# bennevans/mjrl

Measured on AMD Instinct MI355X. Metric: NPG train_step timesteps/sec, Humanoid 1M-step batch @ 1/2/4/8 MI355X, higher is better.
Workload: dtype f32 (split-f16 MFMA, f32 accumulate); 1 GPU; humanoid_npg_1M; obs_dim=376, act_dim=17, algo=npg, horizon=1000, cg_iters=10, parallelism=dp1, comm=LocalComm

## Files before the change

### include/mjrl_amd.h

```cpp
#ifndef MJRL_AMD_H
#define MJRL_AMD_H

#include <stdint.h>

#ifdef __cplusplus
extern "C" {
#endif

#define MJRL_OK 0
#define MJRL_EINVAL (-1)
#define MJRL_ESHAPE (-2)

typedef struct mjrl_shape {
    int32_t n, m;
    int32_t h0, h1;
    int32_t np, mp;
    int32_t d;
    int32_t packed;
} mjrl_shape;

typedef struct mjrl_rows {
    int64_t T;
    const float* xhat;
    const float* act;
// ... 88 lines not shown
int mjrl_quadratic_baseline_gram_scratch(int32_t n, int64_t T, int64_t* doubles);
int mjrl_quadratic_baseline_gram(const double* obs, const double* returns, int64_t T, int32_t n,
                                 const int64_t* path_off, int64_t P, double* scratch, double* out, void* stream);
int mjrl_quadratic_baseline_gram_f32(const float* obs, const float* obs_lo, const double* returns, int64_t T,
                                     int32_t n, const int64_t* path_off, int64_t P, double* scratch, double* out,
                                     void* stream);
int mjrl_quadratic_baseline_residual(const double* obs, const double* returns, int64_t T, int32_t n,
                                     const int64_t* path_off, int64_t P, const double* coeffs, double* scratch,
                                     double* out, void* stream);
int mjrl_quadratic_baseline_residual_f32(const float* obs, const float* obs_lo, const double* returns, int64_t T,
                                         int32_t n, const int64_t* path_off, int64_t P, const double* coeffs,
                                         double* scratch, double* out, void* stream);

int mjrl_gather_rows(const void* src, int64_t row_bytes, const int64_t* idx, int64_t n, void* dst,
                     void* stream);

int mjrl_moments(const double* x, int64_t N, const double* center, double* rpart,
                 double* out, void* stream);
int mjrl_moments_f32(const float* x, int64_t N, const double* center, double* rpart,
                     double* out, void* stream);

#define MJRL_MOM_SCRATCH 2056
int mjrl_moments2(const double* x1, int64_t N1, const double* c1, const double* x2, int64_t N2,
                  const double* c2, double* rpart, double* out1, double* out2, void* stream);
int mjrl_whiten_moments(const double* adv, int64_t T, const double* m1, const double* m2, double eps,
                        float* adv32, double* w64, double* rpart, double* out, void* stream);

int mjrl_moments_combine(const double* gathered, int32_t world, int32_t rec, int32_t ngroups, double* out,
                         void* stream);

int mjrl_whiten(const double* adv, int64_t T, const double* m1, const double* m2,
                double eps, float* adv32, double* w64, void* stream);

int mjrl_dapg_adv(const double* w64, int64_t T, const double* mw1, const double* mw2,
                  int64_t T_demo, double demo_coef, float* adv_vpg, void* stream);

int mjrl_pack_params(const mjrl_shape* s, const float* theta, float* packed,
                     int32_t clamp_log_std, float min_log_std, void* stream);

int mjrl_policy_vpg(const mjrl_shape* s, const mjrl_rows* rows, const float* packed_theta,
                    const float* out_shift, const float* out_scale,
                    const mjrl_scratch* sc, float* gsum, void* stream);
int mjrl_policy_fvp(const mjrl_shape* s, const mjrl_rows* rows, int64_t T_fvp,
                    const float* packed_theta, const float* packed_v,
                    const float* out_scale, const mjrl_scratch* sc, const int32_t* done,
                    float* gsum, void* stream);
int mjrl_policy_eval(const mjrl_shape* s, const mjrl_rows* rows, int64_t T_eval,
                     const float* packed_theta_new, const float* packed_theta_old,
                     const float* out_shift, const float* out_scale,
                     const mjrl_scratch* sc, double* sums, void* stream);
int mjrl_policy_eval_if(const mjrl_shape* s, const mjrl_rows* rows, int64_t T_eval, const float* packed_theta_new,
                        const float* packed_theta_old, const float* out_shift, const float* out_scale,
                        const mjrl_scratch* sc, double* sums, const int32_t* skip, void* stream);

int mjrl_vpg_accumulate(const mjrl_shape* s, const mjrl_rows* rows, const float* packed_theta,
                        const float* out_shift, const float* out_scale, const mjrl_scratch* sc,
                        void* stream);
int mjrl_vpg_accumulate_pack(const mjrl_shape* s, const mjrl_rows* rows, const float* obs,
                             const float* packed_theta, const float* out_shift, const float* out_scale,
                             const mjrl_scratch* sc, void* stream);
int mjrl_policy_vpg_pack(const mjrl_shape* s, const mjrl_rows* rows, const float* obs,
                         const float* packed_theta, const float* out_shift, const float* out_scale,
                         const mjrl_scratch* sc, float* gsum, void* stream);
int mjrl_fvp_accumulate(const mjrl_shape* s, const mjrl_rows* rows, int64_t T_fvp,
                        const float* packed_theta, const float* packed_v, const float* out_scale,
                        const int32_t* done, const mjrl_scratch* sc, void* stream);
int mjrl_gather_grads(const mjrl_shape* s, const mjrl_rows* rows, int64_t T,
                      const mjrl_scratch* sc, int32_t with_log_std, const int32_t* done,
                      float* gsum, void* stream);
int mjrl_fused_path(const mjrl_shape* s);

#define MJRL_CG_STATE 4096
int mjrl_cg_init(const mjrl_shape* s, const float* b, float* x, float* r, float* p,
                 float* packed_p, float* cg, int32_t* done, void* stream);
int mjrl_cg_init_scaled(const mjrl_shape* s, const float* gsum, double scale, float* g, float* x, float* r, float* p,
                        float* packed_p, float* cg, int32_t* done, void* stream);
int mjrl_cg_step(const mjrl_shape* s, const float* gsum, double inv_T, float damping,
                 const float* packed_theta, float* x, float* r, float* p, float* z,
                 float* packed_p, float* cg, int32_t* done, float residual_tol,
                 void* stream);

int mjrl_gather_cg_z(const mjrl_shape* s, const mjrl_rows* rows, int64_t T, const mjrl_scratch* sc,
                     const int32_t* done, float* gsum, double inv_T, float damping,
                     const float* packed_theta, const float* p, float* z, float* cg, void* stream);
int mjrl_cg_step_xr_p(const mjrl_shape* s, float* x, const float* r, float* r_out, float* p,
                      const float* z, float* packed_p, float* cg, int32_t* done, float residual_tol,
                      void* stream);

int mjrl_cg_z(const mjrl_shape* s, const float* gsum, double inv_T, float damping, const float* packed_theta,
              const float* p, float* z, float* cg, const int32_t* done, void* stream);

int mjrl_cg_step1(const mjrl_shape* s, const float* gsum, double inv_T, float damping,
                  const float* packed_theta, float* x, const float* r, float* r_out, const float* p,
                  float* p_out, float* packed_p, float* cg, int32_t* done, float residual_tol,
                  void* stream);

int mjrl_cg_init_vec(int32_t d, const float* b, float* x, float* r, float* p, float* cg,
                     int32_t* done, void* stream);
int mjrl_cg_update(int32_t d, const float* z, float* x, float* r, float* p, float* cg,
                   int32_t* done, float residual_tol, void* stream);

int mjrl_scale_vec(const float* gsum, int32_t d, double scale, float* g, void* stream);

#define MJRL_STEP_OUT 1024
int mjrl_npg_step(const mjrl_shape* s, const float* g, const float* x, const float* theta,
                  int32_t mode, float delta, float alpha_in, int32_t const_lr,
// ... 78 lines not shown
```

### mjrl_amd/_lib.py

```python
import ctypes as C
import os

import torch

HERE = os.path.dirname(os.path.abspath(__file__))
LIB_PATH = os.path.join(HERE, "lib", "libmjrl_amd.so")

MJRL_OK = 0
MJRL_EINVAL = -1
MJRL_ESHAPE = -2
CG_STATE = 4096
CG_PZ_PARTS = 1024
STEP_OUT = 1024
LS_LOG, LS_STATE = 32, 128
MOM_SCRATCH = 2056


class Shape(C.Structure):
    _fields_ = [("n", C.c_int32), ("m", C.c_int32), ("h0", C.c_int32), ("h1", C.c_int32),
                ("np", C.c_int32), ("mp", C.c_int32), ("d", C.c_int32), ("packed", C.c_int32)]


class Rows(C.Structure):
    _fields_ = [("T", C.c_int64)] + [(k, C.c_void_p) for k in (
# ... 12 lines not shown
    _fields_ = [("p", C.c_void_p * 7), ("exp_avg", C.c_void_p * 7), ("exp_avg_sq", C.c_void_p * 7)]


class PolicyFitData(C.Structure):
    _fields_ = [(k, C.c_void_p) for k in ("obs", "act", "adv", "ll_old", "old_log_std", "in_shift", "in_scale",
                                          "out_shift", "out_scale")] + \
               [("T", C.c_int64), ("n", C.c_int32), ("m", C.c_int32), ("h0", C.c_int32), ("h1", C.c_int32),
                ("kind", C.c_int32), ("clip", C.c_double)]


POLICY_FIT_BC, POLICY_FIT_PPO = 0, 1


class Adam(C.Structure):
    _fields_ = [("lr", C.c_double), ("beta1", C.c_double), ("beta2", C.c_double), ("eps", C.c_double),
                ("weight_decay", C.c_double), ("step0", C.c_int64)]


P = C.c_void_p
I32 = C.c_int32
I64 = C.c_int64
F32 = C.c_float
F64 = C.c_double
SP = C.POINTER(Shape)

SIGNATURES = {
    "mjrl_shape_init": [SP, I32, I32, I32, I32],
    "mjrl_scratch_size": [SP, I64, C.POINTER(I64), C.POINTER(I64), C.POINTER(I32)],
    "mjrl_pack_batch": [P, P, I64, SP, P, P, P, P, P],
    "mjrl_obs_colscale": [P, I64, SP, P, P, P, P],
    "mjrl_obs_colscale_f32": [P, I64, SP, P, P, P, P],
    "mjrl_obs_colscale_range": [P, P, SP, P, P, P, P],
    "mjrl_pack_batch_split": [P, P, I64, SP, P, P, P, P, P, P, P],
    "mjrl_pack_batch_f32": [P, P, I64, SP, P, P, P, P, P],
    "mjrl_pack_batch_split_f32": [P, P, I64, SP, P, P, P, P, P, P, P],
    "mjrl_split_supported": [SP],
    "mjrl_gae": [P, P, P, P, I64, F64, F64, I32, P, P, P, P],
    "mjrl_gae_wave": [P, P, P, P, I64, F64, F64, I32, P, P, P, P],
    "mjrl_gae_scan": [P, P, P, P, I64, F64, F64, I32, P, P, P, P],
    "mjrl_linear_baseline": [P, I64, I32, P, I64, P, P, P],
    "mjrl_linear_baseline_f32": [P, I64, I32, P, I64, P, P, P],
    "mjrl_moments": [P, I64, P, P, P, P],
    "mjrl_moments_f32": [P, I64, P, P, P, P],
    "mjrl_moments2": [P, I64, P, P, I64, P, P, P, P, P],
    "mjrl_whiten_moments": [P, I64, P, P, F64, P, P, P, P, P],
    "mjrl_moments_combine": [P, I32, I32, I32, P, P],
    "mjrl_whiten": [P, I64, P, P, F64, P, P, P],
    "mjrl_dapg_adv": [P, I64, P, P, I64, F64, P, P],
    "mjrl_pack_params": [SP, P, P, I32, F32, P],
    "mjrl_policy_vpg": [SP, C.POINTER(Rows), P, P, P, C.POINTER(Scratch), P, P],
    "mjrl_policy_fvp": [SP, C.POINTER(Rows), I64, P, P, P, C.POINTER(Scratch), P, P, P],
    "mjrl_policy_eval": [SP, C.POINTER(Rows), I64, P, P, P, P, C.POINTER(Scratch), P, P],
    "mjrl_policy_eval_if": [SP, C.POINTER(Rows), I64, P, P, P, P, C.POINTER(Scratch), P, P, P],
    "mjrl_vpg_accumulate": [SP, C.POINTER(Rows), P, P, P, C.POINTER(Scratch), P],
    "mjrl_vpg_accumulate_pack": [SP, C.POINTER(Rows), P, P, P, P, C.POINTER(Scratch), P],
    "mjrl_policy_vpg_pack": [SP, C.POINTER(Rows), P, P, P, P, C.POINTER(Scratch), P, P],
    "mjrl_fvp_accumulate": [SP, C.POINTER(Rows), I64, P, P, P, P, C.POINTER(Scratch), P],
    "mjrl_gather_grads": [SP, C.POINTER(Rows), I64, C.POINTER(Scratch), I32, P, P, P],
    "mjrl_fused_path": [SP],
    "mjrl_cg_init": [SP, P, P, P, P, P, P, P, P],
    "mjrl_cg_init_scaled": [SP, P, F64, P, P, P, P, P, P, P, P],
    "mjrl_cg_step": [SP, P, F64, F32, P, P, P, P, P, P, P, P, F32, P],
    "mjrl_gather_cg_z": [SP, C.POINTER(Rows), I64, C.POINTER(Scratch), P, P, F64, F32, P, P, P, P, P],
    "mjrl_cg_step_xr_p": [SP, P, P, P, P, P, P, P, P, F32, P],
    "mjrl_cg_z": [SP, P, F64, F32, P, P, P, P, P, P],
    "mjrl_cg_step1": [SP, P, F64, F32, P, P, P, P, P, P, P, P, P, F32, P],
    "mjrl_cg_init_vec": [I32, P, P, P, P, P, P, P],
    "mjrl_cg_update": [I32, P, P, P, P, P, P, F32, P],
    "mjrl_scale_vec": [P, I32, F64, P, P],
    "mjrl_gather_rows": [P, I64, P, I64, P, P],
    "mjrl_linear_baseline_gram_scratch": [I32, I64, C.POINTER(I64)],
    "mjrl_linear_baseline_gram": [P, P, I64, I32, P, I64, P, P, P],
    "mjrl_linear_baseline_residual": [P, P, I64, I32, P, I64, P, P, P, P],
    "mjrl_linear_baseline_gram_f32": [P, P, I64, I32, P, I64, P, P, P],
    "mjrl_linear_baseline_residual_f32": [P, P, I64, I32, P, I64, P, P, P, P],
    "mjrl_linear_baseline_gram_f32x2": [P, P, P, I64, I32, P, I64, P, P, P],
    "mjrl_linear_baseline_residual_f32x2": [P, P, P, I64, I32, P, I64, P, P, P, P],
    "mjrl_quadratic_baseline_gram_scratch": [I32, I64, C.POINTER(I64)],
    "mjrl_quadratic_baseline_gram": [P, P, I64, I32, P, I64, P, P, P],
    "mjrl_quadratic_baseline_gram_f32": [P, P, P, I64, I32, P, I64, P, P, P],
    "mjrl_quadratic_baseline_residual": [P, P, I64, I32, P, I64, P, P, P, P],
    "mjrl_quadratic_baseline_residual_f32": [P, P, P, I64, I32, P, I64, P, P, P, P],
    "mjrl_npg_step": [SP, P, P, P, I32, F32, F32, I32, F32, P, P, P, P],
    "mjrl_trpo_trial": [SP, P, P, F32, P, P, P, P, F64, F64, I32, I32, P, P, P],
    "mjrl_policy_mean": [SP, P, I64, P, P, P, P, P, P, P],
    "mjrl_policy_mean_slots": [SP, P, P, I64, I64, P, P, P, P, P, P, P],
    "mjrl_value_features_slots": [P, P, P, I64, I64, I32, I64, P, P],
    "mjrl_value_features_finish": [P, P, I64, I32, I64, I64, P, P, P],
    "mjrl_value_mlp_scratch": [I32, I32, C.POINTER(I64)],
    "mjrl_value_mlp_epoch": [P, P, I64, I32, P, I64, I32, C.POINTER(ValueNet), C.POINTER(Adam), P, P, P, P],
    "mjrl_policy_fit_scratch": [I32, I32, I32, I32, I32, C.POINTER(I64)],
    "mjrl_policy_fit_epoch": [C.POINTER(PolicyFitData), P, I64, I32, C.POINTER(PolicyNet), C.POINTER(Adam), P, I32,
                              P, P, P],
    "mjrl_build_flags": [],
    "mjrl_host_stage_f64": [P, I64, I32, P, P, P],
    "mjrl_host_stage_f32": [P, I64, I32, P, P, P],
    "mjrl_host_stage_paths_f64": [P, P, I32, I32, P, P, P],
    "mjrl_host_stage_paths_f64x": [P, P, I32, I32, P, P, P, P, P, I32, P],
    "mjrl_host_stage_lo_paths_f64": [P, P, I32, I32, P],
    "mjrl_host_extras_portable": [P, I64, I32, P, P, P],
    "mjrl_host_stage_rows_f64x": [P, I64, I32, P, P, P, P, P, P, P],
    "mjrl_host_stage_f64_portable": [P, I64, I32, P, P, P],
    "mjrl_host_stage_avx512": [],
    "mjrl_host_gather": [P, P, I32, P],
}

# ... 13 lines not shown
    if not os.path.isabs(path) and not os.path.exists(path):
        path = os.path.join(os.path.dirname(HERE), path)
    if not os.path.exists(path):
        raise MjrlError("mjrl_amd HIP library not built: %s (run `python -m mjrl_amd.build`)" % path)
    lib = C.CDLL(path)
    for name, args in SIGNATURES.items():
        fn = getattr(lib, name)
        fn.argtypes = args
        fn.restype = C.c_int
    if lib.mjrl_build_flags() & BUILD_ABLATION and os.environ.get("MJRL_AMD_ALLOW_ABLATION") != "1":
        raise MjrlError("%s is a timing-ablation build (MJRL_KX_ABL_*: its results are wrong by construction); "
                        "set MJRL_AMD_ALLOW_ABLATION=1 to load it for timing" % path)
    _LIB = lib
    return lib


STAGE_LIB_PATH = os.path.join(HERE, "lib", "libmjrl_stage.so")
STAGE_FUNCS = ("mjrl_host_stage_f64", "mjrl_host_stage_f32", "mjrl_host_stage_paths_f64",
               "mjrl_host_stage_paths_f64x", "mjrl_host_stage_lo_paths_f64", "mjrl_host_extras_portable",
               "mjrl_host_stage_rows_f64x",
               "mjrl_host_stage_f64_portable", "mjrl_host_stage_avx512", "mjrl_host_gather")
_STAGE = None


def stage_lib():
    global _STAGE
    if _STAGE is None:
        if not os.path.exists(STAGE_LIB_PATH):
            raise MjrlError("mjrl_amd staging library not built: %s (run `python -m mjrl_amd.build`)"
                            % STAGE_LIB_PATH)
        lib = C.CDLL(STAGE_LIB_PATH)
        for name in STAGE_FUNCS:
            fn = getattr(lib, name)
            fn.argtypes = SIGNATURES[name]
            fn.restype = C.c_int
        _STAGE = lib
    return _STAGE


def lib():
    if not torch.cuda.is_available():
        raise MjrlError("mjrl_amd needs an AMD GPU (torch.cuda.is_available() is False); "
                        "there is no CPU fallback")
    return load()


def check(rc, what):
    if rc != MJRL_OK:
        msg = {MJRL_EINVAL: "invalid argument", MJRL_ESHAPE: "unsupported policy shape"}.get(
            rc, "HIP error %d" % rc)
        raise MjrlError("%s failed: %s" % (what, msg))


QUERIES = ("mjrl_fused_path", "mjrl_split_supported", "mjrl_build_flags", "mjrl_host_stage_avx512")
_CALLS = {}


class _DevPtr:

    @staticmethod
    def from_param(v, _T=torch.Tensor, _vp=C.c_void_p):
        if type(v) is _T:
            return _vp(v.data_ptr())
        if v is None or type(v) is _vp:
            return v
        if isinstance(v, _T):
            return _vp(v.data_ptr())
        return _vp.from_param(v)


class _HostPtr:

    @staticmethod
    def from_param(v, _vp=C.c_void_p):
        c = getattr(v, "ctypes", None)
        return _vp(c.data) if c is not None else _DevPtr.from_param(v)


def _errcheck(rc, fn, args):
    if rc:
        check(rc, fn.__name__)
    return rc


def _checked(path, names, ptr):
    h = _CALLS.get(path)
    if h is None:
        h = _CALLS[path] = C.CDLL(path)
        for name in names:
            fn = getattr(h, name)
            fn.argtypes = [ptr if a is P else a for a in SIGNATURES[name]]
            fn.restype = C.c_int
            if name not in QUERIES:
                fn.errcheck = _errcheck
    return h


def calls(loader=lib):
    return _checked(loader()._name, SIGNATURES, _DevPtr)


def stage_calls():
    return _checked(stage_lib()._name, STAGE_FUNCS, _HostPtr)


def make_shape(n, m, h0, h1, loader=load):
    s = Shape()
# ... 13 lines not shown
```

### mjrl_amd/csrc/policy.hip

```cpp
#include <math.h>
#include <stdlib.h>

#include "common.h"

using namespace mjrl;

namespace {

enum { FWD = 0, FVP = 1, EVAL = 2 };

struct RowArgs {
    int64_t T;
    int np, m;
    const float* xhat;
    const float* act;
    const float* adv;
    const float* adv_vpg;
    float* a0;
    float* a1;
    float* mu0;
    float* ll0;
    float* gu0;
    float* gu1;
    float* gp;
// ... 961 lines not shown
        const int s0 = w * per, s1 = min(S, s0 + per);
        const float* p = wpart + (int64_t)blockIdx.x * S * 64 + lane;
        if (s1 > s0) MJRL_SLAB_CHECK((int64_t)blockIdx.x * S * 64 + lane + (int64_t)(s1 - 1) * 64, wcap);
        for (int sb = s0; sb < s1; sb += GATHER_PER) {
            float v[GATHER_PER];
#pragma unroll
            for (int j = 0; j < GATHER_PER; ++j) v[j] = sb + j < s1 ? p[(int64_t)(sb + j) * 64] : 0.f;
#pragma unroll
            for (int j = 0; j < GATHER_PER; ++j) acc += (double)v[j];
        }
    } else if (f < d && lspart) {
        const int lsj = f - d_mu;
        const int per = (G + GATHER_WAVES - 1) / GATHER_WAVES;
        const int b0 = w * per, b1 = min(G, b0 + per);
        for (int b = b0; b < b1; ++b) acc += lspart[(int64_t)b * mp + lsj];
    }
    part[w][lane] = acc;
    if (done && *done) return;
    __syncthreads();
    if (w == 0) {
        float gs = 0.f;
        if (f < d) {
            double t = part[0][lane];
#pragma unroll
            for (int j = 1; j < GATHER_WAVES; ++j) t += part[j][lane];
            gs = (float)t;
            gsum[f] = gs;
        }
        if (cz.p) cgz_epilogue(cz, f, d, gs, pf, lsv);
    }
}

__global__ void __launch_bounds__(64) k_eval_final(const double* __restrict__ rpart, int G, double* __restrict__ sums,
                                                   const int32_t* __restrict__ skip) {
    if (skip && *skip) return;
    double s = 0.0, k = 0.0;
    for (int b = threadIdx.x; b < G; b += 64) {
        s += rpart[2 * b];
        k += rpart[2 * b + 1];
    }
    s = wave_sum(s);
    k = wave_sum(k);
    if (threadIdx.x == 0) {
        sums[0] = s;
        sums[1] = k;
    }
}

}

#include "fused.h"
#include "ks.h"
#include "kx.h"

namespace {

constexpr int ROW_GRID_CAP = 512;
constexpr int WGRAD_SLICES_CAP = 128;

inline int bt_for(int h0, int h1) { return rows_bt(h0 > h1 ? h0 : h1); }

inline int row_grid(const mjrl_shape* s, int64_t T) {
    const int bt = bt_for(s->h0, s->h1);
    int64_t nt = (T + bt - 1) / bt;
    if (nt < 1) nt = 1;
    return (int)(nt < ROW_GRID_CAP ? nt : ROW_GRID_CAP);
}

inline int wgrad_slices(int64_t T) {
    int64_t nt = (T + WT - 1) / WT;
    if (nt < 1) nt = 1;
    return (int)(nt < WGRAD_SLICES_CAP ? nt : WGRAD_SLICES_CAP);
}

struct JobSet {
    int njobs;
    WJob job[3];
    int64_t floats;
};

int64_t slab_floats(const mjrl_shape* s, int S);

JobSet make_jobs(const mjrl_shape* s, const mjrl_rows* r, int S) {
    JobSet js{};
    auto add = [&](const float* G, int ldg, const float* A, int lda, int N, int K, int bias) {
        WJob& j = js.job[js.njobs++];
        j.G = G; j.ldg = ldg; j.A = A; j.lda = lda; j.N = N; j.K = K;
        j.nbN = (N + WB - 1) / WB; j.nbK = (K + WB - 1) / WB; j.bias = bias;
        j.off = js.floats;
        js.floats += (int64_t)S * N * K;
        j.boff = js.floats;
        if (bias) js.floats += (int64_t)S * N;
    };
    if (s->h0 == 0) {
        add(r ? r->gp : nullptr, s->mp, r ? r->xhat : nullptr, s->np, s->mp, s->np, 0);
    } else {
        add(r ? r->gu0 : nullptr, s->h0, r ? r->xhat : nullptr, s->np, s->h0, s->np, 0);
        add(r ? r->gu1 : nullptr, s->h1, r ? r->a0 : nullptr, s->h0, s->h1, s->h0, 1);
        add(r ? r->gp : nullptr, s->mp, r ? r->a1 : nullptr, s->h1, s->mp, s->h1, 1);
    }
    return js;
}

template <int H0, int H1, int MP, int MODE>
int launch_rows_t(const RowArgs& ra, int grid, hipStream_t st) {
    using L = Layout<H0, H1, MP>;
// ... 83 lines not shown
    static const bool v = getenv("MJRL_AMD_WGRAD_OLD") && getenv("MJRL_AMD_WGRAD_OLD")[0] == '1';
    return v;
}
bool wall_supported(const mjrl_shape* s) {
    if (wall_off() || s->h0 == 0 || s->h0 != s->h1 || s->np % 16 || !wall_npbm(s)) return false;
    if (s->mp != 16 && s->mp != 32 && s->mp != 64) return false;
    if (s->h0 == 128 && s->mp == 64 && wall_npbm(s) == 8) return false;
    return s->h0 == 128 || ((s->h0 == 32 || s->h0 == 64) && s->mp == 64);
}
inline int wall_cap(const mjrl_shape*) { return 256; }
inline int wall_slices(const mjrl_shape* s, int64_t T) {
    const int bt = 32;
    int64_t tiles = (T + bt - 1) / bt;
    if (tiles < 1) tiles = 1;
    const int cap = wall_cap(s);
    const int64_t tps = (tiles + cap - 1) / cap;
    return (int)((tiles + tps - 1) / tps);
}
inline int rows_slices(const mjrl_shape* s, int64_t T) { return wall_supported(s) ? wall_slices(s, T) : wgrad_slices(T); }

inline int grad_slices(const mjrl_shape* s, int64_t T) {
    const int p = acc_path(s, T);
    return p == 2 ? ks_grid(T) : (p == 1 ? fused_grid(T) : rows_slices(s, T));
}

bool ksx_supported(const mjrl_shape* s) { return ks_supported(s) && s->np % 128 == 0; }

template <int MP, int KG, int MODE>
int launch_ks_t(const RowArgs& ra, const FOut& fo, int grid, hipStream_t st) {
    using L = KLayout<MP, KG>;
    auto fn = k_ks<MP, KG, MODE>;
    static bool attr = false;
    if (!attr) {
        hipError_t e = hipFuncSetAttribute((const void*)fn, hipFuncAttributeMaxDynamicSharedMemorySize, L::bytes);
        if (e != hipSuccess) return (int)e;
        attr = true;
    }
    hipLaunchKernelGGL(fn, dim3(grid), dim3(KT), L::bytes, st, ra, fo);
    return (int)hipGetLastError();
}

template <int MP, int KG, int MODE, bool PACK = false>
int launch_kx_t(const RowArgs& ra, const FOut& fo, int grid, hipStream_t st) {
    using L = XLayout<MP, KG>;
    auto fn = k_kx<MP, KG, MODE, PACK>;
    static bool attr = false;
    if (!attr) {
        hipError_t e = hipFuncSetAttribute((const void*)fn, hipFuncAttributeMaxDynamicSharedMemorySize, L::bytes);
        if (e != hipSuccess) return (int)e;
        attr = true;
    }
    hipLaunchKernelGGL(fn, dim3(grid), dim3(KT), L::bytes, st, ra, fo);
    return (int)hipGetLastError();
}

template <int MODE>
int launch_ks(const mjrl_shape* s, const RowArgs& ra, const FOut& fo, int grid, hipStream_t st) {
    const int kg = s->np / 32;
    if (ra.xs) {
#define MJRL_K(MP_, KG_) \
    if (s->mp == MP_ && kg == KG_) return launch_kx_t<MP_, KG_, MODE>(ra, fo, grid, st);
#define MJRL_KN(MP_) MJRL_K(MP_, 4) MJRL_K(MP_, 8) MJRL_K(MP_, 12)
        MJRL_KN(16)
        MJRL_KN(32)
#undef MJRL_KN
#undef MJRL_K
        return MJRL_ESHAPE;
    }
#define MJRL_K(MP_, KG_) \
    if (s->mp == MP_ && kg == KG_) return launch_ks_t<MP_, KG_, MODE>(ra, fo, grid, st);
#define MJRL_KN(MP_) MJRL_K(MP_, 2) MJRL_K(MP_, 4) MJRL_K(MP_, 6) MJRL_K(MP_, 8) MJRL_K(MP_, 12)
    MJRL_KN(16)
    MJRL_KN(32)
#undef MJRL_KN
#undef MJRL_K
    return MJRL_ESHAPE;
}

template <int H, int MP, int NCH, int MODE>
int launch_fused_t(const RowArgs& ra, const FOut& fo, int grid, hipStream_t st) {
    using L = FLayout<H, H, MP, NCH, MODE>;
    auto fn = k_fused<H, H, MP, NCH, MODE>;
    static bool attr = false;
    if (!attr) {
        hipError_t e = hipFuncSetAttribute((const void*)fn, hipFuncAttributeMaxDynamicSharedMemorySize, L::bytes);
        if (e != hipSuccess) return (int)e;
        attr = true;
    }
    hipLaunchKernelGGL(fn, dim3(grid), dim3(FT), L::bytes, st, ra, fo);
    return (int)hipGetLastError();
}

template <int MODE>
int launch_fused(const mjrl_shape* s, const RowArgs& ra, const FOut& fo, int grid, hipStream_t st) {
    const int nch = (s->np + 63) / 64;
#define MJRL_F(H_, MP_, N_) \
    if (s->h0 == H_ && s->mp == MP_ && nch == N_) return launch_fused_t<H_, MP_, N_, MODE>(ra, fo, grid, st);
#define MJRL_FN(H_, MP_) MJRL_F(H_, MP_, 1) MJRL_F(H_, MP_, 2) MJRL_F(H_, MP_, 3) MJRL_F(H_, MP_, 4) \
    MJRL_F(H_, MP_, 5) MJRL_F(H_, MP_, 6)
    MJRL_FN(64, 16)
    MJRL_FN(64, 32)
    MJRL_FN(32, 16)
    MJRL_FN(32, 32)
#undef MJRL_FN
#undef MJRL_F
    return MJRL_ESHAPE;
// ... 287 lines not shown
    ra.P = packed_theta;
    ra.V = packed_v;
    ra.out_scale = out_scale;
    ra.done = done;
    if (T_fvp == 0) {
        hipMemsetAsync(sc->wpart, 0, slab_floats(s, grad_slices(s, 0)) * sizeof(float), st);
        return (int)hipGetLastError();
    }
    if (acc_path(s, T_fvp)) return run_fused(FVP, s, rows, T_fvp, ra, sc, st);
    int e = launch_rows<FVP>(s, ra, row_grid(s, T_fvp), st);
    if (e) return e;
    return run_wgrad_only(s, rows, T_fvp, sc, done, st);
}

int mjrl_gather_grads(const mjrl_shape* s, const mjrl_rows* rows, int64_t T, const mjrl_scratch* sc,
                      int32_t with_log_std, const int32_t* done, float* gsum, void* stream) {
    if (!rows_ok(s, rows) || !sc || !gsum || T < 0 || T > rows->T) return MJRL_EINVAL;
    if (!shape_supported(s->h0, s->h1, s->mp)) return MJRL_ESHAPE;
    return run_gather(s, rows, T, sc, with_log_std ? sc->rpart : nullptr, done, gsum, (hipStream_t)stream);
}

int mjrl_policy_vpg(const mjrl_shape* s, const mjrl_rows* rows, const float* packed_theta, const float* out_shift,
                    const float* out_scale, const mjrl_scratch* sc, float* gsum, void* stream) {
    int e = mjrl_vpg_accumulate(s, rows, packed_theta, out_shift, out_scale, sc, stream);
    if (e) return e;
    return mjrl_gather_grads(s, rows, rows->T, sc, 1, nullptr, gsum, stream);
}

int mjrl_policy_fvp(const mjrl_shape* s, const mjrl_rows* rows, int64_t T_fvp, const float* packed_theta,
                    const float* packed_v, const float* out_scale, const mjrl_scratch* sc, const int32_t* done,
                    float* gsum, void* stream) {
    if (!sc || !gsum) return MJRL_EINVAL;
    int e = mjrl_fvp_accumulate(s, rows, T_fvp, packed_theta, packed_v, out_scale, done, sc, stream);
    if (e) return e;
    return mjrl_gather_grads(s, rows, T_fvp, sc, 0, done, gsum, stream);
}

int mjrl_gather_cg_z(const mjrl_shape* s, const mjrl_rows* rows, int64_t T, const mjrl_scratch* sc,
                     const int32_t* done, float* gsum, double inv_T, float damping, const float* packed_theta,
                     const float* p, float* z, float* cg, void* stream) {
    if (!rows_ok(s, rows) || !sc || !gsum || !packed_theta || !p || !z || !cg || T < 0 || T > rows->T)
        return MJRL_EINVAL;
    if (!shape_supported(s->h0, s->h1, s->mp)) return MJRL_ESHAPE;
    if ((s->d + 63) / 64 > (MJRL_CG_STATE - CG_PZ_PARTS) / 2) return MJRL_EINVAL;
    const Packed pk(s->h0, s->h1, s->np, s->mp);
    CgZ cz{p, z, cg, packed_theta + pk.ls, inv_T, damping, s->d - s->m};
    return run_gather(s, rows, T, sc, nullptr, done, gsum, (hipStream_t)stream, cz);
}

int mjrl_fused_path(const mjrl_shape* s) { return s ? acc_path(s, 1) : 0; }

int mjrl_split_supported(const mjrl_shape* s) { return s && ksx_supported(s) ? 1 : 0; }

static int policy_eval(const mjrl_shape* s, const mjrl_rows* rows, int64_t T_eval, const float* packed_theta_new,
                       const float* packed_theta_old, const float* out_shift, const float* out_scale,
                       const mjrl_scratch* sc, double* sums, const int32_t* skip, void* stream);

int mjrl_policy_eval(const mjrl_shape* s, const mjrl_rows* rows, int64_t T_eval, const float* packed_theta_new,
                     const float* packed_theta_old, const float* out_shift, const float* out_scale,
                     const mjrl_scratch* sc, double* sums, void* stream) {
    return policy_eval(s, rows, T_eval, packed_theta_new, packed_theta_old, out_shift, out_scale, sc, sums, nullptr,
                       stream);
}

int mjrl_policy_eval_if(const mjrl_shape* s, const mjrl_rows* rows, int64_t T_eval, const float* packed_theta_new,
                        const float* packed_theta_old, const float* out_shift, const float* out_scale,
                        const mjrl_scratch* sc, double* sums, const int32_t* skip, void* stream) {
    if (!skip) return MJRL_EINVAL;
    return policy_eval(s, rows, T_eval, packed_theta_new, packed_theta_old, out_shift, out_scale, sc, sums, skip,
                       stream);
}

static int policy_eval(const mjrl_shape* s, const mjrl_rows* rows, int64_t T_eval, const float* packed_theta_new,
                       const float* packed_theta_old, const float* out_shift, const float* out_scale,
                       const mjrl_scratch* sc, double* sums, const int32_t* skip, void* stream) {
    if (!rows_ok(s, rows) || !packed_theta_new || !packed_theta_old || !sc || !sums || T_eval < 0 ||
        T_eval > rows->T || !rows->adv || !rows->mu0 || !rows->ll0)
        return MJRL_EINVAL;
    if (!shape_supported(s->h0, s->h1, s->mp)) return MJRL_ESHAPE;
    hipStream_t st = (hipStream_t)stream;
    RowArgs ra = row_args(s, rows, T_eval);
    ra.P = packed_theta_new;
    ra.V = packed_theta_old;
    ra.out_shift = out_shift;
    ra.out_scale = out_scale;
    ra.rpart = sc->rpart;
    ra.done = skip;
    const bool ks = ks_supported(s);
    const int G = ks ? ks_grid(T_eval) : row_grid(s, T_eval);
    if (T_eval > 0) {
        int e = ks ? launch_ks<EVAL>(s, ra, FOut{}, G, st) : launch_rows<EVAL>(s, ra, G, st);
        if (e) return e;
    } else {
        hipMemsetAsync(sc->rpart, 0, sizeof(double) * 2 * G, st);
    }
    hipLaunchKernelGGL(k_eval_final, dim3(1), dim3(64), 0, st, sc->rpart, G, sums, skip);
    return (int)hipGetLastError();
}

}
```

### mjrl_amd/engine.py

```python
import collections
import ctypes as C
import functools
import math
import os

import time

import numpy as np
import torch

from . import _lib
from ._capture import capture
from .comm import LocalComm

S_M1, S_M2, S_PM1, S_PM2, S_MS, S_EVAL, S_MW1, S_MW2 = 0, 8, 16, 24, 32, 38, 40, 48
N_STATS = 64


def _thread_safe_predict(baseline):
    return type(baseline).__name__ in ("QuadraticBaseline", "ZeroBaseline", "LinearBaseline")


def _linear_coeffs(baseline, n):
    if baseline is None or type(baseline).__name__ != "LinearBaseline" or not hasattr(baseline, "_coeffs"):
# ... 402 lines not shown
            base = None
            adv = stage("adv", [p["advantages"] for p in paths], 0)
        elif coeffs is not False and hpred is not None:
            base = hpred
            adv = None
        elif coeffs is not False:
            base = _STAGING.device_slot("base", T, np.float64, device) if reuse else \
                torch.empty(T, dtype=torch.float64, device=device)
            base.zero_()
            if coeffs is not None and T > 0:
                c = torch.from_numpy(np.ascontiguousarray(coeffs, dtype=np.float64)).to(device)
                K = _lib.calls()
                fn = K.mjrl_linear_baseline_f32 if obs.dtype == torch.float32 else K.mjrl_linear_baseline
                fn(obs, T, n, off, len(paths), c, base, _lib.stream_ptr())
            adv = None
        elif hasattr(baseline, "predict_device"):
            base = baseline.predict_device(obs, off, lengths)
            adv = None
        else:
            preds = list(_STAGING.pool().map(
                lambda p: baseline.predict(p) if baseline is not None else np.zeros(len(p["rewards"])), paths)) \
                if baseline is not None and _thread_safe_predict(baseline) else \
                [baseline.predict(p) if baseline is not None else np.zeros(len(p["rewards"])) for p in paths]
            base = stage("base", preds, 0)
            adv = None
        b = cls(obs, act, rew, base, off, term, advantages=adv, T_demo=T_demo, obs_range=orange)
        b.lengths = lengths
        b.obs_inexact = inexact
        if pre is not None and pre.get("obs_lo") is not None and inexact:
            b._obs_lo = pre["obs_lo"]
        return b

    def obs_lo(self, paths=None, reuse=True):
        if not self.obs_inexact or self.obs.dtype != torch.float32:
            return None
        lo = getattr(self, "_obs_lo_dev", None)
        if lo is not None:
            return lo
        src = getattr(self, "_obs_lo", None)
        dev = self.obs.device
        with torch.cuda.device(dev):
            if src is not None:
                lo = _STAGING.stage_host("obs_lo", src, dev, reuse)
            else:
                if paths is None or sum(len(p["rewards"]) for p in paths) != self.T:
                    raise ValueError("DeviceBatch.obs_lo needs the batch's RL paths")
                lo = _STAGING.stage("obs_lo", [p["observations"] for p in paths], self.obs.shape[1], np.float32, dev,
                                    reuse, low=True)
        self._obs_lo_dev = lo
        return lo


FUSED_PACK = os.environ.get("MJRL_AMD_FUSED_PACK", "1") != "0"
TRPO_DEVICE_TRIALS = int(os.environ.get("MJRL_AMD_TRPO_DEVICE_TRIALS", "4"))
GRAPH_AUTO_ROWS = 300_000
HIDDEN_WIDTHS = (32, 64, 128, 256)


def kernel_hidden(n, m, hidden):
    if m < 1 or m > 64:
        raise ValueError("mjrl_amd kernels support act_dim 1..64, got %d" % m)
    if n < 1:
        raise ValueError("obs_dim must be positive")
    if hidden is None or tuple(hidden) == (0, 0):
        return (0, 0)
    hidden = tuple(int(h) for h in hidden)
    if len(hidden) != 2 or min(hidden) < 1:
        raise ValueError("the Gaussian MLP has two hidden layers (gaussian_mlp.py:143-158), got %r" % (hidden,))
    for w in HIDDEN_WIDTHS:
        if max(hidden) <= w:
            return (w, w)
    raise ValueError("mjrl_amd kernels support hidden sizes up to %d, got %r" % (HIDDEN_WIDTHS[-1], hidden))


def padded_positions(n, m, hidden, kh):
    h0, h1 = hidden
    p0, p1 = kh
    o_b0 = p0 * n
    o_w1 = o_b0 + p0
    o_b1 = o_w1 + p1 * p0
    o_w2 = o_b1 + p1
    o_b2 = o_w2 + m * p1
    o_ls = o_b2 + m
    parts = [(np.arange(h0)[:, None] * n + np.arange(n)[None, :]).ravel(),
             o_b0 + np.arange(h0),
             (o_w1 + np.arange(h1)[:, None] * p0 + np.arange(h0)[None, :]).ravel(),
             o_b1 + np.arange(h1),
             (o_w2 + np.arange(m)[:, None] * p1 + np.arange(h1)[None, :]).ravel(),
             o_b2 + np.arange(m),
             o_ls + np.arange(m)]
    return np.concatenate(parts).astype(np.int64)


class UpdateEngine:

    def __init__(self, n, m, hidden, device=None, comm=None, min_log_std=-3.0, precision=None):
        self.lib = _lib.lib()
        self.K = _lib.calls()
        real = (0, 0) if hidden is None else (int(hidden[0]), int(hidden[1]))
        kh = kernel_hidden(int(n), int(m), hidden)
        self.shape = _lib.make_shape(int(n), int(m), *kh)
        self.device = torch.device(device if device is not None else "cuda")
        self.hidden = real
        self.pad_idx = None
        if kh != real:
            self.pad_idx = torch.from_numpy(padded_positions(int(n), int(m), real, kh)).to(self.device)
            self._pad_bufs = {}
        self.comm = comm or LocalComm()
        self.min_log_std = float(min_log_std)
        self.cap_T = -1
        self.cap_P = -1
        s = self.shape
        dev = self.device
        f32 = dict(dtype=torch.float32, device=dev)
        self.packed_theta = torch.zeros(s.packed, **f32)
        self.packed_new = torch.zeros(s.packed, **f32)
        self.packed_p = torch.zeros(s.packed, **f32)
        self.pvec = {k: torch.zeros(s.d, **f32) for k in ("g", "gsum", "x", "r", "r2", "p", "p2", "z", "theta_new")}
        self.cg = torch.zeros(_lib.CG_STATE, **f32)
        self.done = torch.zeros(1, dtype=torch.int32, device=dev)
        self.out = torch.zeros(_lib.STEP_OUT, **f32)
        self.stats = torch.zeros(N_STATS, dtype=torch.float64, device=dev)
        self.mom_part = torch.zeros(4 * 256 + 16, dtype=torch.float64, device=dev)
        self.mom2_part = torch.zeros(_lib.MOM_SCRATCH, dtype=torch.float64, device=dev)
        self.transforms = (None, None, None, None)
        self._act_rows = None
        self.trpo_device_trials = TRPO_DEVICE_TRIALS
        self.ls_state = torch.zeros(_lib.LS_STATE, **f32)
        self.ls_skip = torch.zeros(1, dtype=torch.int32, device=dev)
        self.sharded = bool(getattr(self.comm, "sharded", self.comm.world_size > 1))
        self.gbuf = torch.zeros(max(self.comm.world_size, 1) * 32, dtype=torch.float64, device=dev)
        self.kernel_timing = None
        self.graphs = "auto"
        self._gstate = {}
        self.gae_mode = os.environ.get("MJRL_AMD_GAE", "serial")
        self.fused = bool(self.K.mjrl_fused_path(self.shape))
        prec = precision or os.environ.get("MJRL_AMD_PRECISION", "auto")
        if prec not in ("auto", "split", "f32"):
            raise ValueError("precision must be 'auto', 'split' or 'f32', got %r" % (prec,))
        can_split = bool(self.K.mjrl_split_supported(self.shape))
        if prec == "split" and not can_split:
            raise ValueError("split precision is not available for this policy shape")
        self.split = can_split and prec != "f32"
        self.precision = "split" if self.split else "f32"

    @property
    def vec(self):
        if self.pad_idx is None:
            return self.pvec
        return {k: t[self.pad_idx] for k, t in self.pvec.items()}

# ... 713 lines not shown
```

Measured before the change: 94.94 million timesteps/s.

## Add software-pipelined eval kernel overlapping next-tile layer-0 MFMA with current tile

Adds a new policy-eval kernel that loads and publishes the next row tile's inputs into double-buffered LDS. It interleaves that tile's first-layer MFMA steps, split across four phases by a configurable sixths split, with the hidden, output and row-pass stages of the current tile. It also prefetches the next tile's act, mu and advantage lines. The aim is to hide global-load latency and keep the matrix units busy during the tanh and reduction phases of the line-search eval. It is enabled by default when split x is available, and can be toggled through an env var or API call. The cost is higher LDS and register pressure, with one block per CU.

```diff
diff --git a/include/mjrl_amd.h b/include/mjrl_amd.h
--- a/include/mjrl_amd.h
+++ b/include/mjrl_amd.h
@@ -164,6 +164,8 @@
 int mjrl_policy_eval_if(const mjrl_shape* s, const mjrl_rows* rows, int64_t T_eval, const float* packed_theta_new,
                         const float* packed_theta_old, const float* out_shift, const float* out_scale,
                         const mjrl_scratch* sc, double* sums, const int32_t* skip, void* stream);
+int mjrl_eval_pipe(int32_t on);
+int mjrl_eval_grid(const mjrl_shape* s, int64_t T_eval);
 
 int mjrl_vpg_accumulate(const mjrl_shape* s, const mjrl_rows* rows, const float* packed_theta,
                         const float* out_shift, const float* out_scale, const mjrl_scratch* sc,
diff --git a/mjrl_amd/_lib.py b/mjrl_amd/_lib.py
--- a/mjrl_amd/_lib.py
+++ b/mjrl_amd/_lib.py
@@ -88,6 +88,8 @@
     "mjrl_policy_fvp": [SP, C.POINTER(Rows), I64, P, P, P, C.POINTER(Scratch), P, P, P],
     "mjrl_policy_eval": [SP, C.POINTER(Rows), I64, P, P, P, P, C.POINTER(Scratch), P, P],
     "mjrl_policy_eval_if": [SP, C.POINTER(Rows), I64, P, P, P, P, C.POINTER(Scratch), P, P, P],
+    "mjrl_eval_pipe": [I32],
+    "mjrl_eval_grid": [SP, I64],
     "mjrl_vpg_accumulate": [SP, C.POINTER(Rows), P, P, P, C.POINTER(Scratch), P],
     "mjrl_vpg_accumulate_pack": [SP, C.POINTER(Rows), P, P, P, P, C.POINTER(Scratch), P],
     "mjrl_policy_vpg_pack": [SP, C.POINTER(Rows), P, P, P, P, C.POINTER(Scratch), P, P],
@@ -207,7 +209,8 @@
         raise MjrlError("%s failed: %s" % (what, msg))
 
 
-QUERIES = ("mjrl_fused_path", "mjrl_split_supported", "mjrl_build_flags", "mjrl_host_stage_avx512")
+QUERIES = ("mjrl_fused_path", "mjrl_split_supported", "mjrl_build_flags", "mjrl_host_stage_avx512",
+           "mjrl_eval_pipe", "mjrl_eval_grid")
 _CALLS = {}
 
 
diff --git a/mjrl_amd/csrc/kxe.h b/mjrl_amd/csrc/kxe.h
--- /dev/null
+++ b/mjrl_amd/csrc/kxe.h
@@ -0,0 +1,345 @@
+#pragma once
+
+namespace {
+
+#ifndef MJRL_KXE_SPLIT
+#define MJRL_KXE_SPLIT 1, 1, 1, 3
+#endif
+template <int MP, int KG>
+struct XELayout {
+    static constexpr int H = 64, BT = 32;
+    static constexpr int NP = 32 * KG, KH = NP / 2;
+    static constexpr int RBYTES = NP * 2;
+    static constexpr int XIMG = BT * RBYTES;
+    static constexpr int LD = H + 4;
+    static constexpr int LDG = 32 + 4;
+    static constexpr int WIMG = 64 * 128;
+    static constexpr int WIMG2 = 32 * 128;
+    static constexpr int AIMG = AIMG_BYTES;
+    static constexpr int oX = 0;
+    static constexpr int oS1 = oX + 4 * XIMG;
+    static constexpr int oS3 = oS1 + 2 * WIMG;
+    static constexpr int oSC = oS3 + 2 * WIMG2;
+    static constexpr int oU = oSC + (64 + 32) * 4;
+    static constexpr int oD0 = oU + 2 * BT * 4;
+    static constexpr int oGP = oD0 + BT * LD * 4;
+    static constexpr int oA0 = oGP + BT * LDG * 4;
+    static constexpr int oA1 = oA0 + 2 * AIMG;
+    static constexpr int bytes = oA1 + 2 * AIMG;
+    static_assert(bytes <= 160 * 1024, "LDS");
+    static_assert(bytes >= 2 * KT * 8, "row_pass_final scratch");
+    static constexpr int XPER = BT * NP / 4 / KT;
+    static constexpr int KS = KH / 32;
+    static_assert(NP % 128 == 0, "chunk swizzle of the xhat images");
+    static_assert(MP == 16 || MP == 32, "output layer: one k32 step");
+    static constexpr int step0(int i) {
+        constexpr int c[4] = {MJRL_KXE_SPLIT};
+        static_assert(c[0] + c[1] + c[2] + c[3] == 6, "MJRL_KXE_SPLIT: sixths");
+        int cum = 0;
+        for (int k = 0; k < i; ++k) cum += c[k];
+        return (KS * cum + 3) / 6;
+    }
+    static constexpr int gmax() {
+        int g = 1;
+        for (int i = 0; i < 4; ++i) g = step0(i + 1) - step0(i) > g ? step0(i + 1) - step0(i) : g;
+        return g;
+    }
+};
+
+template <int MP, int KG>
+__global__ void __launch_bounds__(KT, 1) k_kx_eval_pipe(RowArgs a) {
+#pragma clang fp contract(fast)
+    using L = XELayout<MP, KG>;
+    constexpr int H = 64, BT = L::BT, NP = L::NP, KH = L::KH, KS = L::KS;
+    extern __shared__ __attribute__((aligned(16))) float smem[];
+    char* sb = reinterpret_cast<char*>(smem);
+    char* S1 = sb + L::oS1;
+    char* S3 = sb + L::oS3;
+    float* sc1 = reinterpret_cast<float*>(sb + L::oSC);
+    float* sc3 = sc1 + 64;
+    float* Us2 = reinterpret_cast<float*>(sb + L::oU);
+    float* D0 = reinterpret_cast<float*>(sb + L::oD0);
+    float* GPf = reinterpret_cast<float*>(sb + L::oGP);
+    char* A0i = sb + L::oA0;
+    char* A1i = sb + L::oA1;
+
+#ifdef MJRL_KX_PROF
+    const unsigned long long kx_t0_ = __builtin_amdgcn_s_memtime();
+    unsigned long long kx_pre_[6];
+#endif
+    const int tid = threadIdx.x, lane = tid & 63, w = __builtin_amdgcn_readfirstlane(tid >> 6);
+    const int r16 = lane & 15, q = lane >> 4;
+    const int cb = w & 3, kh = w >> 2;
+    const int m = a.m;
+    const int64_t T = a.T;
+    const int64_t ntiles = (T + BT - 1) / BT;
+    const int64_t G = gridDim.x;
+    const float* P = a.P;
+    const Packed pk(H, H, NP, MP);
+
+    static_assert(KT == 512 && MP <= 32, "preamble layout: 8 waves, output-layer images of 32 rows");
+    const float8v rv1 = wload_rows<64>(P + pk.W1, H, tid);
+    const float8v rv2 = wload_rows<32>(P + pk.W2, MP, tid);
+    const float bias1 = P[pk.b1 + cb * 16 + r16];
+    const int cbo3 = w & (MP / 16 - 1), rb3 = w / (MP / 16);
+    const int col3 = cbo3 * 16 + r16;
+    const float bias3 = P[pk.b2 + col3];
+    const float os3 = a.out_scale ? (col3 < m ? a.out_scale[col3] : 1.f) : 1.f;
+    const float osh3 = a.out_shift ? (col3 < m ? a.out_shift[col3] : 0.f) : 0.f;
+    const float sls = ls_sum(P + pk.ls, m);
+    const RowConst rconst = row_const<EVAL, MP>(a, P + pk.ls, tid);
+    KX_PRE(0);
+    half8 wh[KS], wl[KS];
+    float wsc;
+    {
+        float8v v[KS];
+#pragma unroll
+        for (int s = 0; s < KS; ++s) {
+            const int k0 = kh * KH + 32 * s + 8 * q;
+            v[s] = load8(P + pk.W0 + (cb * 16 + r16) * NP + k0) * load8(a.xc + k0);
+        }
+        float mx = 0.f;
+#pragma unroll
+        for (int s = 0; s < KS; ++s) mx = fmaxf(mx, absmax8(v[s]));
+        const float sc = pow2_scale(max_over_groups(mx), wsc);
+#pragma unroll
+        for (int s = 0; s < KS; ++s) split8(v[s], sc, wh[s], wl[s]);
+    }
+    KX_PRE(1);
+    wrows_store<64>(rv1, S1, L::WIMG, sc1, tid);
+    wrows_store<32>(rv2, S3, L::WIMG2, sc3, tid);
+    KX_PRE(2);
+    KX_PRE(3);
+    KX_PRE(4);
+    if (a.done && *a.done) return;
+
+    double racc0 = 0.0, racc1 = 0.0;
+    float touch[2] = {0.f, 0.f};
+    float4 xn[L::XPER];
+    float un = 1.f;
+    auto xload = [&](int64_t t_, int u0 = 0, int u1 = L::XPER) {
+        const int64_t rb_ = t_ * BT;
+        const int row = tid >> 4, c16 = tid & 15;
+        const bool ok = t_ < ntiles && rb_ + row < T;
+        const char* src = reinterpret_cast<const char*>(a.xs) + (ok ? (rb_ + row) * (4 * NP) : 0);
+#pragma unroll
+        for (int u = 0; u < L::XPER; ++u)
+            if (u >= u0 && u < u1)
+                xn[u] = ok ? *reinterpret_cast<const float4*>(src + 16 * (c16 + 16 * u)) : make_float4(0.f, 0.f, 0.f, 0.f);
+        if (u0 == 0) {
+            const bool uok = tid < BT && t_ < ntiles && rb_ + tid < T;
+            un = a.xu[uok ? rb_ + tid : 0];
+        }
+    };
+    auto publish = [&](int b) {
+        const int row = tid >> 4, c16 = tid & 15;
+        char* dst = sb + L::oX + b * (2 * L::XIMG) + row * L::RBYTES + 16 * (c16 ^ chunk_swz(row));
+#pragma unroll
+        for (int u = 0; u < L::XPER; ++u) {
+            constexpr int UH = NP / 128;
+            *reinterpret_cast<float4*>(dst + (u / UH) * L::XIMG + 256 * (u % UH)) = xn[u];
+        }
+        if (tid < BT) Us2[b * BT + tid] = un;
+    };
+    const int p1A = 16 * (kh * (KH / 8) + q), p1B = 16 * chunk_swz(r16), p1C = r16 * L::RBYTES;
+    constexpr int GMAX = L::gmax();
+    auto p1_load = [&](int b, int s0, int s1, half8 (&xh)[GMAX][2], half8 (&xl)[GMAX][2]) __attribute__((always_inline)) {
+        const char* XH = sb + L::oX + b * (2 * L::XIMG);
+#pragma unroll
+        for (int s = 0; s < KS; ++s)
+            if (s >= s0 && s < s1) {
+#pragma unroll
+                for (int i = 0; i < 2; ++i) {
+                    const int off = ((p1A + 64 * s) ^ p1B) + p1C + i * 16 * L::RBYTES;
+                    xh[s - s0][i] = *reinterpret_cast<const half8*>(XH + off);
+                    xl[s - s0][i] = *reinterpret_cast<const half8*>(XH + L::XIMG + off);
+                }
+            }
+    };
+    auto p1_mma = [&](int s0, int s1, const half8 (&xh)[GMAX][2], const half8 (&xl)[GMAX][2], floatx4 (&acc)[2])
+        __attribute__((always_inline)) {
+#pragma unroll
+        for (int s = 0; s < KS; ++s)
+            if (s >= s0 && s < s1) {
+#pragma unroll
+                for (int i = 0; i < 2; ++i) acc[i] = mfma_x3(xh[s - s0][i], xl[s - s0][i], wh[s], wl[s], acc[i]);
+            }
+    };
+    auto p1_steps = [&](int b, int s0, int s1, floatx4 (&acc)[2]) __attribute__((always_inline)) {
+#pragma unroll
+        for (int g0 = 0; g0 < KS; g0 += GMAX) {
+            half8 xh[GMAX][2], xl[GMAX][2];
+            const int lo = g0 > s0 ? g0 : s0, hi = g0 + GMAX < s1 ? g0 + GMAX : s1;
+            p1_load(b, lo, hi, xh, xl);
+            p1_mma(lo, hi, xh, xl, acc);
+        }
+    };
+    auto p1_scale = [&](int b, floatx4 (&acc)[2]) __attribute__((always_inline)) {
+#pragma unroll
+        for (int i = 0; i < 2; ++i)
+#pragma unroll
+            for (int rr = 0; rr < 4; ++rr) acc[i][rr] *= Us2[b * BT + i * 16 + 4 * q + rr] * wsc;
+    };
+
+    xload(blockIdx.x);
+    __syncthreads();
+    publish(0);
+    xload(blockIdx.x + G);
+    __syncthreads();
+    floatx4 acc1[2] = {zero4(), zero4()};
+    p1_steps(0, 0, KS, acc1);
+    p1_scale(0, acc1);
+#ifdef MJRL_KX_PROF
+    unsigned long long kx_acc_[KX_NPROF] = {0};
+    unsigned long long kx_last_ = __builtin_amdgcn_s_memtime();
+    kx_acc_[15] = kx_last_ - kx_t0_;
+    kx_acc_[17] = 1;
+    kx_acc_[18] = kx_pre_[0] - kx_t0_;
+    for (int i = 1; i < 5; ++i) kx_acc_[18 + i] = kx_pre_[i] - kx_pre_[i - 1];
+    kx_acc_[23] = kx_last_ - kx_pre_[4];
+#endif
+
+    int nb = 1;
+    for (int64_t tile = blockIdx.x; tile < ntiles; tile += G) {
+        KX_STAMP(9);
+        const int64_t row_base = tile * BT;
+
+#pragma unroll
+        for (int rr = 0; rr < 4; ++rr)
+            D0[((1 - kh) * 16 + 4 * q + rr) * L::LD + cb * 16 + r16] = kh ? acc1[0][rr] : acc1[1][rr];
+        asm volatile("" ::"v"(touch[0]), "v"(touch[1]));
+        publish(nb);
+        {
+            const int64_t nt = tile + G;
+            if (nt < ntiles) {
+                const int64_t nbase = nt * BT;
+                const int nr = (int)(T - nbase < BT ? T - nbase : BT);
+                const int mline = (BT * m * 4 + 127) / 128;
+                const int idx = tid;
+                const float* p = nullptr;
+                const int ne = nr * m;
+                if (idx < mline) {
+                    if (32 * idx < ne) p = a.act + nbase * m + 32 * idx;
+                } else if (idx < 2 * mline) {
+                    if (32 * (idx - mline) < ne) p = a.mu0 + nbase * m + 32 * (idx - mline);
+                } else if (idx == 2 * mline) {
+                    p = a.adv + nbase;
+                } else if (idx == 2 * mline + 1) {
+                    p = a.ll0 + nbase;
+                }
+                touch[0] = *(p ? p : reinterpret_cast<const float*>(a.xs));
+            } else {
+                touch[0] = *reinterpret_cast<const float*>(a.xs);
+            }
+        }
+        __syncthreads();
+        KX_STAMP(0);
+
+        half8 ph[GMAX][2], pl[GMAX][2];
+
+        floatx4 accn[2] = {zero4(), zero4()};
+        {
+            const int col = cb * 16 + r16;
+            float dv[4];
+#pragma unroll
+            for (int rr = 0; rr < 4; ++rr) dv[rr] = D0[(kh * 16 + 4 * q + rr) * L::LD + col];
+            p1_load(nb, L::step0(0), L::step0(1), ph, pl);
+            __builtin_amdgcn_sched_barrier(0);
+            float av[4];
+#pragma unroll
+            for (int rr = 0; rr < 4; ++rr) av[rr] = tanhf((kh ? acc1[1][rr] : acc1[0][rr]) + dv[rr]);
+            astore4(A0i, col, kh * 16 + 4 * q, av);
+            p1_mma(L::step0(0), L::step0(1), ph, pl, accn);
+        }
+        xload(tile + 2 * G, 0, L::XPER / 2);
+        __builtin_amdgcn_sched_barrier(0);
+        __syncthreads();
+        KX_STAMP(2);
+
+        {
+            const int j = cb * 16 + r16;
+            half8 bh[2], bl[2], xh[2], xl[2];
+#pragma unroll
+            for (int s = 0; s < 2; ++s) {
+                arow(A0i, kh, s, q, r16, xh[s], xl[s]);
+                wrow(S1, L::WIMG, j, s, q, bh[s], bl[s]);
+            }
+            const float rsc = sc1[j] * AHR_INV;
+            p1_load(nb, L::step0(1), L::step0(2), ph, pl);
+            __builtin_amdgcn_sched_barrier(0);
+            floatx4 acc = zero4();
+#pragma unroll
+            for (int s = 0; s < 2; ++s) acc = mfma_x3(xh[s], xl[s], bh[s], bl[s], acc);
+#pragma unroll
+            for (int rr = 0; rr < 4; ++rr) acc[rr] *= rsc;
+            float av[4];
+#pragma unroll
+            for (int rr = 0; rr < 4; ++rr) {
+                const float v = acc[rr] + bias1;
+                av[rr] = tanhf(v);
+            }
+            astore4(A1i, j, kh * 16 + 4 * q, av);
+            p1_mma(L::step0(1), L::step0(2), ph, pl, accn);
+        }
+        xload(tile + 2 * G, L::XPER / 2, L::XPER);
+        __builtin_amdgcn_sched_barrier(0);
+        __syncthreads();
+        KX_STAMP(3);
+
+        RowPre<BT, MP, KT> rpre;
+        row_pre_load<EVAL, BT, MP, KT>(a, row_base, tid, rpre);
+        {
+            const bool p3 = w < 2 * (MP / 16);
+            half8 bh[2], bl[2], xh[2], xl[2];
+            float rsc = 0.f;
+            if (p3) {
+#pragma unroll
+                for (int s = 0; s < 2; ++s) {
+                    arow(A1i, rb3, s, q, r16, xh[s], xl[s]);
+                    wrow(S3, L::WIMG2, col3, s, q, bh[s], bl[s]);
+                }
+                rsc = sc3[col3] * AHR_INV;
+            }
+            p1_load(nb, L::step0(2), L::step0(3), ph, pl);
+            __builtin_amdgcn_sched_barrier(0);
+            if (p3) {
+                floatx4 acc = zero4();
+#pragma unroll
+                for (int s = 0; s < 2; ++s) acc = mfma_x3(xh[s], xl[s], bh[s], bl[s], acc);
+#pragma unroll
+                for (int rr = 0; rr < 4; ++rr) acc[rr] *= rsc;
+#pragma unroll
+                for (int rr = 0; rr < 4; ++rr) {
+                    const int row = rb3 * 16 + 4 * q + rr;
+                    const float v = acc[rr] + bias3;
+                    GPf[row * L::LDG + col3] = col3 < m ? v * os3 + osh3 : 0.f;
+                }
+            }
+            p1_mma(L::step0(2), L::step0(3), ph, pl, accn);
+        }
+        __builtin_amdgcn_sched_barrier(0);
+        __syncthreads();
+        KX_STAMP(4);
+
+        p1_load(nb, L::step0(3), KS, ph, pl);
+        __builtin_amdgcn_sched_barrier(0);
+        row_pass<EVAL, BT, MP, KT, false, true>(a, P + pk.ls, sls, row_base, GPf, L::LDG, racc0, racc1, tid, &rpre,
+                                                &rconst);
+        p1_mma(L::step0(3), KS, ph, pl, accn);
+        p1_scale(nb, accn);
+        acc1[0] = accn[0];
+        acc1[1] = accn[1];
+        nb ^= 1;
+        KX_STAMP(5);
+    }
+
+    __syncthreads();
+    row_pass_final<EVAL, MP, KT>(racc0, racc1, reinterpret_cast<double*>(smem), a.rpart, blockIdx.x, tid);
+#ifdef MJRL_KX_PROF
+    kx_acc_[16] = __builtin_amdgcn_s_memtime() - kx_last_;
+    if (blockIdx.x == 0 && tid == 0)
+        for (int i = 0; i < KX_NPROF; ++i) g_kx_prof[i] += kx_acc_[i];
+#endif
+}
+
+}
diff --git a/mjrl_amd/csrc/policy.hip b/mjrl_amd/csrc/policy.hip
--- a/mjrl_amd/csrc/policy.hip
+++ b/mjrl_amd/csrc/policy.hip
@@ -1037,6 +1037,7 @@
 #include "fused.h"
 #include "ks.h"
 #include "kx.h"
+#include "kxe.h"
 
 namespace {
 
@@ -1226,6 +1227,34 @@
     }
     hipLaunchKernelGGL(fn, dim3(grid), dim3(KT), L::bytes, st, ra, fo);
     return (int)hipGetLastError();
+}
+
+int g_eval_pipe = 1;
+
+template <int MP, int KG>
+int launch_kx_eval_pipe_t(const RowArgs& ra, int grid, hipStream_t st) {
+    using L = XELayout<MP, KG>;
+    auto fn = k_kx_eval_pipe<MP, KG>;
+    static bool attr = false;
+    if (!attr) {
+        hipError_t e = hipFuncSetAttribute((const void*)fn, hipFuncAttributeMaxDynamicSharedMemorySize, L::bytes);
+        if (e != hipSuccess) return (int)e;
+        attr = true;
+    }
+    hipLaunchKernelGGL(fn, dim3(grid), dim3(KT), L::bytes, st, ra);
+    return (int)hipGetLastError();
+}
+
+int launch_kx_eval_pipe(const mjrl_shape* s, const RowArgs& ra, int grid, hipStream_t st) {
+    const int kg = s->np / 32;
+#define MJRL_K(MP_, KG_) \
+    if (s->mp == MP_ && kg == KG_) return launch_kx_eval_pipe_t<MP_, KG_>(ra, grid, st);
+#define MJRL_KN(MP_) MJRL_K(MP_, 4) MJRL_K(MP_, 8) MJRL_K(MP_, 12)
+    MJRL_KN(16)
+    MJRL_KN(32)
+#undef MJRL_KN
+#undef MJRL_K
+    return MJRL_ESHAPE;
 }
 
 template <int MODE>
@@ -1619,6 +1648,17 @@
 
 int mjrl_split_supported(const mjrl_shape* s) { return s && ksx_supported(s) ? 1 : 0; }
 
+int mjrl_eval_pipe(int32_t on) {
+    const int was = g_eval_pipe;
+    if (on >= 0) g_eval_pipe = on != 0;
+    return was;
+}
+
+int mjrl_eval_grid(const mjrl_shape* s, int64_t T_eval) {
+    if (!s || T_eval < 0) return 0;
+    return ks_supported(s) ? ks_grid(T_eval) : row_grid(s, T_eval);
+}
+
 static int policy_eval(const mjrl_shape* s, const mjrl_rows* rows, int64_t T_eval, const float* packed_theta_new,
                        const float* packed_theta_old, const float* out_shift, const float* out_scale,
                        const mjrl_scratch* sc, double* sums, const int32_t* skip, void* stream);
@@ -1656,7 +1696,8 @@
     const bool ks = ks_supported(s);
     const int G = ks ? ks_grid(T_eval) : row_grid(s, T_eval);
     if (T_eval > 0) {
-        int e = ks ? launch_ks<EVAL>(s, ra, FOut{}, G, st) : launch_rows<EVAL>(s, ra, G, st);
+        int e = ks ? (ra.xs && g_eval_pipe ? launch_kx_eval_pipe(s, ra, G, st) : launch_ks<EVAL>(s, ra, FOut{}, G, st))
+                   : launch_rows<EVAL>(s, ra, G, st);
         if (e) return e;
     } else {
         hipMemsetAsync(sc->rpart, 0, sizeof(double) * 2 * G, st);
diff --git a/mjrl_amd/engine.py b/mjrl_amd/engine.py
--- a/mjrl_amd/engine.py
+++ b/mjrl_amd/engine.py
@@ -478,6 +478,7 @@
 
 
 FUSED_PACK = os.environ.get("MJRL_AMD_FUSED_PACK", "1") != "0"
+EVAL_PIPE = os.environ.get("MJRL_AMD_EVAL_PIPE")
 TRPO_DEVICE_TRIALS = int(os.environ.get("MJRL_AMD_TRPO_DEVICE_TRIALS", "4"))
 GRAPH_AUTO_ROWS = 300_000
 HIDDEN_WIDTHS = (32, 64, 128, 256)
@@ -523,6 +524,8 @@
     def __init__(self, n, m, hidden, device=None, comm=None, min_log_std=-3.0, precision=None):
         self.lib = _lib.lib()
         self.K = _lib.calls()
+        if EVAL_PIPE is not None:
+            self.K.mjrl_eval_pipe(int(EVAL_PIPE != "0"))
         real = (0, 0) if hidden is None else (int(hidden[0]), int(hidden[1]))
         kh = kernel_hidden(int(n), int(m), hidden)
         self.shape = _lib.make_shape(int(n), int(m), *kh)
```

Result: faster. 96.05 million timesteps/s, median of 6 (+1.2%).
